# duckdb-faiss-ext/duckdb-faiss-ext

Hardware: AMD Instinct MI355X
Metric: queries/sec, FlatL2 d=128 N=10000000 nq=10000 k=10 (higher is better)
Workload: dtype f32 results (bf16 matrix-pipe coarse filter with a proven bound + exact f32 re-scoring of the candidates); 1 GPU; Flat L2 d=128 N=10000000 nq=10000 k=10; queries_per_call=10000, replicas=1, exchange=none

## Files before the change

### duckdb-faiss-ext_amd/csrc/common.h

```cpp
#pragma once
#include <hip/hip_runtime.h>

#include <cfloat>
#include <cstdint>
#include <cstdio>
#include <stdexcept>
#include <string>

namespace mvs {

struct Error : std::runtime_error {
	explicit Error(const std::string &m) : std::runtime_error(m) {
	}
};

[[noreturn]] void throw_faiss(const char *func, const char *file, const char *fmt, ...);

void ensure_dynamic_lds(const void *kernel, size_t bytes);

#define MVS_HIP(expr)                                                                                                  \
	do {                                                                                                               \
		hipError_t e_ = (expr);                                                                                        \
		if (e_ != hipSuccess)                                                                                          \
			::mvs::throw_faiss(__func__, __FILE__, "HIP error %d (%s) in %s", (int)e_, hipGetErrorString(e_), #expr);  \
// ... 91 lines not shown
                      int64_t nq, const unsigned short *d_rows_bf, const float *d_norms, int64_t n, int64_t kp, float *d_pd,
                      int32_t *d_pi, unsigned *d_gthr, hipStream_t st);
void launch_rescore_verify(int metric, const float *d_ca, const int64_t *d_ci, int64_t nq, int kp, int kk, const float *d_x,
                           const FlatGeom &g, const float *d_vecs, const float *d_norms, const float *d_qn,
                           const unsigned *d_max_norm_bits, float *d_pd1, int32_t *d_pi1, int *d_fail_cnt, int *d_fail_q,
                           unsigned *d_max_rel_err_bits, hipStream_t st);
void launch_gather_query_rows(const float *d_x, int d, const int *d_fq, int nf, float *d_xf, hipStream_t st);
void launch_scatter_rows(const int *d_fq, int nf, int64_t k, const float *d_Df, const int64_t *d_If, float *d_D,
                         int64_t *d_I, hipStream_t st);

constexpr int CL_OUTL_CAP = 256;
struct IvfFlatArith {
	const float *qn;
	const float *yn;
	const long long *rowids;
};

struct Tuning {
	int coarse_mfma = 2;
	int coarse_select = 1;
	int coarse_bf16 = 1;
	int cl_bound_mode = 1;
	int cl_tab = 1;
	int mfma_nsplit = 0;
	int mfma_global_lists = 1;
	int ivf_cl_xcd = 1;
};
const Tuning &tune();
void set_current_tuning(const Tuning *t);
void forget_current_tuning(const Tuning *t);

void trace_push(const char *name);
void trace_pop();
struct TraceRange {
	explicit TraceRange(const char *name) {
		trace_push(name);
	}
	~TraceRange() {
		trace_pop();
	}
	TraceRange(const TraceRange &) = delete;
	TraceRange &operator=(const TraceRange &) = delete;
};

struct DirectPlan {
	int nsplit;
// ... 106 lines not shown
```

### duckdb-faiss-ext_amd/csrc/flat_collect.h

```cpp
#pragma once
#include "flat_fused.h"

namespace mvs {

typedef __bf16 bf16x8 __attribute__((ext_vector_type(8)));
typedef float f32x4n __attribute__((ext_vector_type(4)));
typedef float f32x2n __attribute__((ext_vector_type(2)));
typedef int i32x4n __attribute__((ext_vector_type(4)));
typedef int i32x2n __attribute__((ext_vector_type(2)));
typedef __attribute__((address_space(3))) float lds_f32c;
typedef __attribute__((address_space(1))) const float glb_f32c;

constexpr int CL_QBLOCK = 512;
constexpr int CL_BN = 32;
constexpr double CL_MFMA_UNITS = 8.0;
constexpr int CL_SUB = 2;
constexpr int CL_QCAP = 2048;
constexpr int CL_FLUSH_EVERY = 2;
constexpr int CL_FROZEN = 256;

struct CollectArgs {
	const void *qf;
	const unsigned short *yb;
	const float *yn;
	const float *e2;
	unsigned *gslot;
	unsigned long long *stream;
	unsigned long long *stream_cnt;
	float *stream_s;
	float *seed_stage;
	const unsigned long long *rowmask;
	long long stream_cap;
	int slot_stride, nclass;
	long long n, row_first, split_rows;
	long long split_len;
	int nq, nqb, nsplit, xcd_map;
	float *pbnd;
	int flags;
	float i8_unit;
};

__device__ __forceinline__ int cl_i8_thr(float p, float inv_unit) {
	const float t = ceilf(p * inv_unit);
	if (!(t == t) || t > 1073741824.f)
		return 0x7fffffff;
	if (t < -1073741824.f)
		return -0x7fffffff;
	return (int)t;
}

int collect_store_dims(int d);
int collect_wide_qblock(int dp1);
int collect_wide_slots(int dp1);
int collect_wide_max_classes(int dp1);
size_t collect_wide_lds_bytes(int dp1);
int collect_wide_block_rows(int dp1);
void launch_collect_wide_range(int dp1, int metric, bool collect, CollectArgs a, int64_t row_first, int64_t row_end,
                               int64_t nsplit_want, int64_t nq, hipStream_t st, int *grid_out, int *nsplit_out);
int collect_big_qblock(int dp1);
size_t collect_big_lds_bytes(int dp1);
void launch_collect_big(int dp1, int metric, bool collect, const CollectArgs &a, int grid, hipStream_t st);
void launch_rows_to_bf16_wide(int metric, const float *d_vecs, int sdp, int interleaved, int d, int dp1, int64_t row0, int64_t nrows,
                              const float *d_mu, unsigned short *d_bf, float *d_beta, const float *d_norms,
                              unsigned *d_max_norm_bits, hipStream_t st, int *d_outl);
void launch_collect_exact_wide(int metric, bool per_pair, unsigned long long *d_sorted, int64_t ncand, const float *d_x, int d,
                               const float *d_vecs, int sdp, int interleaved, const float *d_norms, const float *d_qn, hipStream_t st,
                               const unsigned long long *d_cnt = nullptr);

__device__ __forceinline__ unsigned skey(float s) {
	return ~f2key(s);
}
__device__ __forceinline__ float skey2f(unsigned k) {
	return key2f(~k);
// ... 4 lines not shown
```

### duckdb-faiss-ext_amd/csrc/flat_collect.hip

```cpp
#include "flat_collect.h"

#include <algorithm>
#include <climits>
#include <cmath>
#include <cstring>
#include <type_traits>

#include <rocprim/device/device_radix_sort.hpp>
#include <rocprim/device/device_segmented_radix_sort.hpp>

namespace mvs {

__global__ __launch_bounds__(256) void collect_colsum_kernel(const float *__restrict__ src, long long nrows, int dp,
                                                            int interleaved, float *__restrict__ sum) {
	const int g8 = dp / 8, rl = threadIdx.x / g8, c8 = threadIdx.x % g8, nrl = 256 / g8;
	float acc[8] = {0.f, 0.f, 0.f, 0.f, 0.f, 0.f, 0.f, 0.f};
	const long long r0 = (long long)blockIdx.x * 1024;
	__shared__ float red[256 * 8];
	const bool idle = rl >= nrl;
	for (long long r = r0 + rl; !idle && r < r0 + 1024 && r < nrows; r += nrl) {
		const float4 s0 = *(const float4 *)(src + (size_t)r * dp + c8 * 8);
		const float4 s1 = *(const float4 *)(src + (size_t)r * dp + c8 * 8 + 4);
		float v[8];
		if (!interleaved) {
// ... 319 lines not shown
}

__global__ void collect_pack_queries_kernel(const float *__restrict__ x, long long nq, int d, int nkb,
                                            const float *__restrict__ mu, float alpha, bf16x8 *__restrict__ qf,
                                            long long total) {
	const long long i = (long long)blockIdx.x * blockDim.x + threadIdx.x;
	if (i >= total)
		return;
	const int lane = (int)(i & 63);
	const long long t = i >> 6;
	const int kb = (int)(t % nkb);
	const long long qblk16 = t / nkb;
	const long long q = qblk16 * 16 + (lane & 15);
	bf16x8 hi;
#pragma unroll
	for (int e = 0; e < 8; ++e) {
		const int kk = kb * 32 + 8 * (lane >> 4) + e;
		hi[e] = (__bf16)((q < nq && kk < d) ? alpha * (x[q * d + kk] - mu[kk]) : 0.f);
	}
	qf[i] = hi;
}
size_t collect_qfrag_bytes(const FlatGeom &g, int64_t nq) {
	(void)g;
	const int64_t nblk16 = (nq + CL_QBLOCK - 1) / CL_QBLOCK * (CL_QBLOCK / 16);
	return (size_t)nblk16 * 4 * 64 * 16;
}
size_t collect_qfrag_bytes_ex(int dp1, int qblock, int64_t nq) {
	const int64_t nblk16 = (nq + qblock - 1) / qblock * (qblock / 16);
	return (size_t)nblk16 * (dp1 / 32) * 64 * 16;
}
void launch_collect_pack_queries_ex(int d, int dp1, int qblock, int metric, const float *d_x, int64_t nq, const float *d_mu,
                                    void *d_qf, hipStream_t st) {
	const int64_t nblk16 = (nq + qblock - 1) / qblock * (qblock / 16);
	const long long total = (long long)nblk16 * (dp1 / 32) * 64;
	hipLaunchKernelGGL(collect_pack_queries_kernel, dim3((unsigned)((total + 255) / 256)), dim3(256), 0, st, d_x,
	                   (long long)nq, d, dp1 / 32, d_mu, metric == METRIC_L2 ? 2.0f : 1.0f, (bf16x8 *)d_qf, total);
	MVS_HIP(hipGetLastError());
}

template <bool IS_L2>
__global__ void collect_bounds_kernel(const float *__restrict__ x, long long nq, int d, const float *__restrict__ mu,
                                      const unsigned *__restrict__ max_norm_bits, float *__restrict__ e2,
                                      int *__restrict__ fail_cnt, int *__restrict__ fail_q, int bound_mode) {
	const long long q = (long long)blockIdx.x * blockDim.x + threadIdx.x;
	if (q >= nq) {
		e2[q] = __uint_as_float(0x7fc00000u);
		return;
// ... 173 lines not shown
			const int kk = kb * 32 + 8 * (lane >> 4) + e;
			hi[e] = (__bf16)((q0 + r < nq && kk < d) ? alpha * (xs[r][kk] - ms[kk]) : 0.f);
		}
		qf[((q0 / 16 + qb) * 4 + kb) * 64 + lane] = hi;
	}
	const unsigned neutral = ~f2key(-FLT_MAX);
	for (int i = tid; i < 64 * stride; i += 256) {
		const long long q = q0 + i / stride;
		if (q < nq)
			gslot[q * stride + (i % stride)] = neutral;
	}
	if (tid < 64 && q0 + tid < nq) {
		ctl_seg[q0 + tid] = 0;
		ctl_seg[nq + q0 + tid] = 0;
	}
	if (blockIdx.x == 0 && tid < 64)
		ctl_hdr[tid] = 0;
}
void launch_collect_query_prep(int metric, const float *d_x, int64_t nq, int d, const float *d_mu, const unsigned *d_max_norm_bits,
                               void *d_qf, float *d_qn, float *d_e2, int *d_fail_cnt, int *d_fail_q, unsigned *d_gslot, int stride,
                               int *d_ctl_hdr, int *d_ctl_seg, hipStream_t st, const unsigned *d_i8_bits, float i8_sa, float i8_unit) {
	if (nq <= 0)
		return;
	const long long nq_frag = (nq + CL_QBLOCK - 1) / CL_QBLOCK * CL_QBLOCK, nq_e2 = (nq + 255) / 256 * 256;
	const dim3 grid((unsigned)(nq_frag / 64));
	const bool i8 = i8_unit > 0.f;
	auto kern = metric == METRIC_L2 ? (i8 ? collect_query_prep_kernel<true, true> : collect_query_prep_kernel<true>)
	                                : (i8 ? collect_query_prep_kernel<false, true> : collect_query_prep_kernel<false>);
	hipLaunchKernelGGL(kern, grid, dim3(256), 0, st, d_x, (long long)nq, d, d_mu, d_max_norm_bits, (bf16x8 *)d_qf, nq_frag, d_qn, d_e2, nq_e2,
	                   d_fail_cnt, d_fail_q, tune().cl_bound_mode, d_gslot, stride, d_ctl_hdr, d_ctl_seg, d_i8_bits, i8_sa, i8_unit);
	MVS_HIP(hipGetLastError());
}

typedef float f32x4acc __attribute__((ext_vector_type(4)));
template <int KCH, bool IS_L2, bool COLLECT, bool SEL = false, int NC = 16, bool I8 = false>
__global__ __launch_bounds__(256, 2) void flat_bf16_collect_kernel(const CollectArgs a) {
	constexpr int DP = KCH * 16;
	constexpr int KB = I8 ? DP / 64 : DP / 32;
	constexpr int PITCH = I8 ? DP : DP * 2;
	constexpr int C = PITCH / 16;
	constexpr int TILE_BYTES = CL_BN * PITCH;
	constexpr int STAGE_BYTES = CL_SUB * TILE_BYTES;
	constexpr int NDMA = STAGE_BYTES / 1024;
	constexpr int DMA_PER_WAVE = NDMA / 4;
	static_assert(C == (I8 ? 8 : 16) && KB == (I8 ? 2 : 4) && NDMA % 4 == 0 && CL_SUB * CL_BN <= 64, "d = 128 geometry");
	typedef typename std::conditional<I8, i32x4n, bf16x8>::type frag_t;
	typedef typename std::conditional<I8, i32x4n, f32x4acc>::type acc_t;
	typedef typename std::conditional<I8, i32x2n, f32x2n>::type bnd_t;
	typedef typename std::conditional<I8, int, float>::type val_t;
	const float unit = a.i8_unit;

	extern __shared__ __attribute__((aligned(16))) float smem[];
	char *tbuf = (char *)smem;
	float *nbuf = (float *)(tbuf + 2 * STAGE_BYTES);
	unsigned long long *qbuf = (unsigned long long *)(nbuf + 2 * 64);
	float *cqtab = (float *)(qbuf + CL_QCAP);
	unsigned *qctl = (unsigned *)(cqtab + CL_QBLOCK);
	float *qval = (float *)(qctl + 16);
	float *cqstage = qval + CL_QCAP;

	const int tid = threadIdx.x, lane = tid & 63;
	const int wave = __builtin_amdgcn_readfirstlane(tid >> 6);
	const int hq = lane >> 4, c = lane & 15;
	int split, qb;
	if (a.xcd_map) {
		const int xcd = blockIdx.x & 7, idx = blockIdx.x >> 3;
		split = (idx / a.nqb) * 8 + xcd;
		qb = idx % a.nqb;
	} else {
		split = blockIdx.x / a.nqb;
		qb = blockIdx.x % a.nqb;
	}
	const long long r_begin = a.row_first + (long long)split * a.split_rows;
	long long r_end = r_begin + a.split_rows;
	if (r_end > a.n)
		r_end = a.n;
	const int ntiles = r_end > r_begin ? (int)((r_end - r_begin + CL_SUB * CL_BN - 1) / (CL_SUB * CL_BN)) : 0;
	if (tid == 0)
		qctl[7] = 0u;

	const int qw = qb * CL_QBLOCK + wave * 128;

	frag_t bq[8][KB];
	{
		const frag_t *qsrc = (const frag_t *)a.qf;
#pragma unroll
		for (int cb = 0; cb < 8; ++cb) {
			const size_t qblk16 = (size_t)qb * (CL_QBLOCK / 16) + wave * 8 + cb;
#pragma unroll
			for (int kb = 0; kb < KB; ++kb)
				bq[cb][kb] = qsrc[(qblk16 * KB + kb) * 64 + lane];
		}
	}

	unsigned dma_off;
	{
		const int rr = I8 ? 8 * wave + (lane >> 3) : 4 * wave + (lane >> 4);
		dma_off = (unsigned)(rr * PITCH + (((lane & (C - 1)) ^ (rr & (C - 1))) * 16));
	}
	auto dma_issue = [&](int u, int i) {
		const char *base = (const char *)a.yb + (size_t)(r_begin + (long long)u * (CL_SUB * CL_BN)) * PITCH + (size_t)i * 4096;
		__builtin_amdgcn_global_load_lds((glb_f32c *)(base + dma_off),
		                                 (lds_f32c *)(smem + ((u & 1) * STAGE_BYTES + (i * 4 + wave) * 1024) / 4), 16, 0, 0);
	};
	auto dma_norms = [&](int u) {
		const float *base = a.yn + (r_begin + (long long)u * (CL_SUB * CL_BN));
		__builtin_amdgcn_global_load_lds((glb_f32c *)(base + lane), (lds_f32c *)(smem + (2 * STAGE_BYTES) / 4 + (u & 1) * 64),
		                                 4, 0, 0);
	};
	const bool use_tab = a.pbnd != nullptr;
	const bool frozen = use_tab && (a.flags & CL_FROZEN) != 0;
	constexpr int tab_shift = 2;
	constexpr int duty_mask = !COLLECT ? 3 : (NC > 32 ? 255 : 63);
	const int duty_phase = split * 13 + 5;
	bool tab_pending = false;
	const float inv_unit = I8 ? 1.0f / unit : 0.f;
	auto dma_bounds = [&]() {
		const float *base = a.pbnd + (size_t)qb * CL_QBLOCK + wave * 128;
		float *dst = (I8 ? cqstage : cqtab) + wave * 128;
		__builtin_amdgcn_global_load_lds((glb_f32c *)(base + lane), (lds_f32c *)dst, 4, 0, 16 );
		__builtin_amdgcn_global_load_lds((glb_f32c *)(base + 64 + lane), (lds_f32c *)(dst + 64), 4, 0, 16);
		tab_pending = I8;
	};
	auto tab_cvt = [&]() {
		if (!I8 || !tab_pending)
			return;
		tab_pending = false;
		const float p0 = cqstage[wave * 128 + lane], p1 = cqstage[wave * 128 + 64 + lane];
		((int *)cqtab)[wave * 128 + lane] = cl_i8_thr(p0, inv_unit);
		((int *)cqtab)[wave * 128 + 64 + lane] = cl_i8_thr(p1, inv_unit);
	};
	if (ntiles > 0) {
#pragma unroll
		for (int i = 0; i < DMA_PER_WAVE; ++i)
			dma_issue(0, i);
		dma_norms(0);
		if (use_tab)
			dma_bounds();
	}
	__syncthreads();
	tab_cvt();

	const unsigned rbase = (unsigned)(c * PITCH) | (unsigned)(((hq ^ c) & (C - 1)) * 16);
	constexpr int WQCAP = CL_QCAP / 4;
	const unsigned qcnt_lds = (unsigned)(uintptr_t)((__attribute__((address_space(3))) unsigned *)qctl);
	const unsigned qbuf_lds = (unsigned)(uintptr_t)((__attribute__((address_space(3))) unsigned long long *)qbuf) + (unsigned)(wave * WQCAP * 8);
	const unsigned qval_lds = (unsigned)(uintptr_t)((__attribute__((address_space(3))) float *)qval) + (unsigned)(wave * WQCAP * 4);
	const unsigned cq_lds = (unsigned)(uintptr_t)((__attribute__((address_space(3))) float *)cqtab) + (unsigned)((wave * 64 + c) * 8);

	int ovf = 0;
	int wfill = 0, wpub = 0;
	auto publish = [&]() __attribute__((always_inline)) {
		const unsigned n = (unsigned)wfill < (unsigned)WQCAP ? (unsigned)wfill : (unsigned)WQCAP;
		for (unsigned e = (unsigned)wpub + lane; e < n && !frozen; e += 64) {
			unsigned long long ent;
			float v;
			asm volatile("ds_read_b64 %0, %2\n\tds_read_b32 %1, %3\n\ts_waitcnt lgkmcnt(0)"
			             : "=&v"(ent), "=&v"(v)
			             : "v"(qbuf_lds + 8u * e), "v"(qval_lds + 4u * e)
			             : "memory");
			const unsigned row = (unsigned)ent;
			typedef __attribute__((address_space(1))) unsigned *GU;
			__hip_atomic_fetch_min((GU)(a.gslot + (size_t)(unsigned)(ent >> 32) * NC) + (row & (unsigned)(NC - 1)), skey(v), __ATOMIC_RELAXED,
			                       __HIP_MEMORY_SCOPE_AGENT);
		}
		wpub = (int)n;
	};
	auto wdrain = [&]() __attribute__((always_inline)) {
		publish();
		const unsigned n = (unsigned)wpub;
		wfill = 0;
// ... 69 lines not shown
				const unsigned long long ent = ((unsigned long long)q << 32) | row;
				if (__builtin_expect(!counting, 1)) {
					asm volatile("ds_write_b64 %0, %1\n\tds_write_b32 %2, %3" ::"v"(qbuf_lds + 8u * pos), "v"(ent), "v"(qval_lds + 4u * pos), "v"(v) : "memory");
				} else {
					typedef __attribute__((address_space(1))) unsigned *GU;
					__hip_atomic_fetch_min((GU)(a.gslot + (size_t)q * NC) + (row & (unsigned)(NC - 1)), skey(v), __ATOMIC_RELAXED,
					                       __HIP_MEMORY_SCOPE_AGENT);
					const unsigned one = 1u;
					asm volatile("ds_add_u32 %0, %1" ::"v"(qcnt_lds + 28u), "v"(one) : "memory");
				}
			}
		}
	};

	for (int u = 0; u < ntiles; ++u) {
		const int period = u < 4 ? 1 : (u < 32 ? 8 : (u < 256 ? 32 : 128));
		const bool full = !frozen && (use_tab ? ((u + duty_phase) & duty_mask) == 0 : (u % period) == 0);
		if (use_tab && !full && u > 0 && (u & ((1 << tab_shift) - 1)) == 0)
			dma_bounds();
		if (full) {
			publish();
			int qo = qw;
			MVS_OPAQUE_VGPR(qo);
			f32x2n v = {0.f, 0.f};
#pragma unroll 1
			for (int i = 0; i < 2; ++i) {
				const int q = qo + 32 * hq + 16 * i + c;
				const int qc = q < a.nq ? q : 0;
				const float e2v = __builtin_nontemporal_load(a.e2 + qc);
				constexpr int SUBN = NC > 32 ? 32 : NC, NSUB = NC / SUBN;
				const int rank = NSUB == 1 ? a.nclass - 1 : (a.nclass + NSUB - 1) / NSUB - 1;
				unsigned kth = 0u;
#pragma unroll 1
				for (int sb = 0; sb < NSUB; ++sb) {
				const unsigned long long *src = (const unsigned long long *)(a.gslot + (size_t)qc * NC + sb * SUBN);
				unsigned long long w[SUBN / 2];
#pragma unroll
				for (int j = 0; j < SUBN / 2; ++j)
					w[j] = __hip_atomic_load(src + j, __ATOMIC_RELAXED, __HIP_MEMORY_SCOPE_AGENT);
#pragma unroll
				for (int j = 0; j < SUBN / 2; ++j)
					asm volatile("" : "+v"(w[j]));
				unsigned key[SUBN];
#pragma unroll
				for (int j = 0; j < SUBN / 2; ++j) {
					key[2 * j] = (unsigned)w[j];
					key[2 * j + 1] = (unsigned)(w[j] >> 32);
				}
#pragma unroll
				for (int kbit = 2; kbit <= SUBN; kbit <<= 1)
// ... 4 lines not shown
							const int x1 = x0 ^ jb;
							if (x1 > x0) {
								const unsigned lo = key[x0] < key[x1] ? key[x0] : key[x1];
								const unsigned hi = key[x0] < key[x1] ? key[x1] : key[x0];
								const bool asc = (x0 & kbit) == 0;
								key[x0] = asc ? lo : hi;
								key[x1] = asc ? hi : lo;
							}
						}
				unsigned ks = key[0];
#pragma unroll
				for (int j = 1; j < SUBN; ++j)
					ks = (rank == j) ? key[j] : ks;
				kth = ks > kth ? ks : kth;
				}
				const unsigned neutral = skey(-FLT_MAX);
				const float B = skey2f(kth < neutral ? kth : neutral);
				const float bv = q < a.nq ? B - e2v : __uint_as_float(0x7fc00000u);
				v[0] = i == 0 ? bv : v[0];
				v[1] = i == 1 ? bv : v[1];
			}
			if (I8) {
				const i32x2n vi = {cl_i8_thr(v[0], inv_unit), cl_i8_thr(v[1], inv_unit)};
				*(i32x2n *)(cqtab + (wave * 64 + hq * 16 + c) * 2) = vi;
			} else {
				*(f32x2n *)(cqtab + (wave * 64 + hq * 16 + c) * 2) = v;
			}
			if (use_tab) {
				unsigned long long bits;
				__builtin_memcpy(&bits, &v, 8);
				__hip_atomic_store((unsigned long long *)(a.pbnd + (size_t)qb * CL_QBLOCK + (wave * 64 + hq * 16 + c) * 2), bits, __ATOMIC_RELAXED,
				                   __HIP_MEMORY_SCOPE_AGENT);
			}
		}
#pragma unroll 1
		for (int sub = 0; sub < CL_SUB; ++sub) {
		frag_t A[KB][2];
		acc_t Y[2];
		{
			const unsigned nb_lds = (unsigned)(uintptr_t)((lds_f32c *)(nbuf + (u & 1) * 64 + sub * CL_BN + 4 * hq));
			asm volatile("ds_read_b128 %0, %2\n\tds_read_b128 %1, %2 offset:64" : "=&v"(Y[0]), "=&v"(Y[1]) : "v"(nb_lds) : "memory");
			const unsigned ab =
			    (unsigned)(uintptr_t)((lds_f32c *)(smem + ((u & 1) * STAGE_BYTES + sub * TILE_BYTES) / 4)) + rbase;
#pragma unroll
			for (int kb = 0; kb < KB; ++kb) {
				asm volatile("ds_read_b128 %0, %1" : "=v"(A[kb][0]) : "v"(ab ^ (unsigned)(kb * 64)) : "memory");
				if (I8)
					asm volatile("ds_read_b128 %0, %1 offset:2048" : "=v"(A[kb][1]) : "v"(ab ^ (unsigned)(kb * 64)) : "memory");
				else
					asm volatile("ds_read_b128 %0, %1 offset:4096" : "=v"(A[kb][1]) : "v"(ab ^ (unsigned)(kb * 64)) : "memory");
			}
		}
		if (sub == 0) {
#pragma unroll
			for (int i = 0; i < DMA_PER_WAVE; ++i)
// ... 12 lines not shown
		bnd_t cqv[2];
		const val_t lowest = I8 ? (val_t)INT_MIN : (val_t)-INFINITY;
		val_t mx0 = lowest, mx1 = lowest;
		auto vmax = [](val_t x, val_t y) {
			if constexpr (I8)
				return x > y ? x : y;
			else
				return __builtin_fmaxf(x, y);
		};
		auto fold = [&](acc_t &p, int rb, int i) {
			(void)rb;
			if (i == 0)
				mx0 = vmax(vmax(vmax(vmax(mx0, p[0]), p[1]), p[2]), p[3]);
			else
				mx1 = vmax(vmax(vmax(vmax(mx1, p[0]), p[1]), p[2]), p[3]);
		};
		auto any_of = [&](bnd_t cqp) {
			const bool r = (mx0 >= cqp[0]) || (mx1 >= cqp[1]);
			mx0 = lowest;
			mx1 = lowest;
			return r;
		};
#pragma unroll
		for (int t = 0; t < 4; ++t) {
			asm volatile("ds_read_b64 %0, %1" : "=v"(cqv[t & 1]) : "v"(cq_lds + (unsigned)(t * 128)) : "memory");
#pragma unroll
			for (int rb = 0; rb < 2; ++rb) {
				const int prb = rb ^ 1, pt = rb == 0 ? t - 1 : t;
#pragma unroll
				for (int kb = 0; kb < KB; ++kb) {
					if constexpr (I8) {
						if (t == 0) {
							if (rb == 0 && kb == 0)
								asm volatile("s_waitcnt lgkmcnt(4)" : "+v"(A[0][0]), "+v"(Y[0]), "+v"(Y[1]));
							else if (rb == 0 && kb == 1)
								asm volatile("s_waitcnt lgkmcnt(2)" : "+v"(A[1][0]));
							else if (rb == 1 && kb == 0)
								asm volatile("s_waitcnt lgkmcnt(0)" : "+v"(A[0][1]), "+v"(A[1][1]), "+v"(cqv[0]));
						}
					} else if (t == 0) {
						if (rb == 0 && kb == 0)
							asm volatile("s_waitcnt lgkmcnt(8)" : "+v"(A[0][0]), "+v"(Y[0]), "+v"(Y[1]));
						else if (rb == 0 && kb == 1)
							asm volatile("s_waitcnt lgkmcnt(6)" : "+v"(A[1][0]));
						else if (rb == 0 && kb == 2)
							asm volatile("s_waitcnt lgkmcnt(4)" : "+v"(A[2][0]));
						else if (rb == 0 && kb == 3)
// ... 4 lines not shown
#pragma unroll
					for (int i = 0; i < 2; ++i) {
						if constexpr (I8)
							acc[rb][i] = __builtin_amdgcn_mfma_i32_16x16x64_i8(A[kb][rb], bq[2 * t + i][kb], kb == 0 ? Y[rb] : acc[rb][i], 0, 0, 0);
						else if (kb == 0)
							acc[rb][i] = __builtin_amdgcn_mfma_f32_16x16x32_bf16(A[kb][rb], bq[2 * t + i][kb], Y[rb], 0, 0, 0);
						else
							acc[rb][i] = __builtin_amdgcn_mfma_f32_16x16x32_bf16(A[kb][rb], bq[2 * t + i][kb], acc[rb][i], 0, 0, 0);
					}
					if (pt >= 0 && kb < 2)
						fold(acc[prb][kb], prb, kb);
					__builtin_amdgcn_sched_barrier(0);
				}
				if (pt >= 0) {
					if (rb == 0)
						asm volatile("s_waitcnt lgkmcnt(0)" : "+v"(cqv[0]), "+v"(cqv[1]));
					rare(acc[prb], prb, pt, any_of(cqv[pt & 1]), cqv[pt & 1], row0, nvalid, rowbits);
				}
			}
		}
		{
			fold(acc[1][0], 1, 0);
			fold(acc[1][1], 1, 1);
			rare(acc[1], 1, 3, any_of(cqv[1]), cqv[1], row0, nvalid, rowbits);
		}
		}
		__syncthreads();
		tab_cvt();
		if ((u % CL_FLUSH_EVERY) == CL_FLUSH_EVERY - 1 || u == ntiles - 1) {
			if (wfill >= WQCAP / 2 || u == ntiles - 1)
				wdrain();
			else
				publish();
		}
	}
	if (COLLECT) {
		__syncthreads();
		if (tid == 0 && qctl[7] != 0u)
			atomicAdd(a.stream_cnt, (unsigned long long)qctl[7]);
	}
}

static size_t collect_lds_bytes(const FlatGeom &g, bool i8) {
	(void)g;
	return (size_t)2 * CL_SUB * CL_BN * 128 * (i8 ? 1 : 2) + 2 * 64 * 4 + (size_t)CL_QCAP * 8 + (size_t)CL_QBLOCK * 4 + 64 + (size_t)CL_QCAP * 4 +
	       (i8 ? (size_t)CL_QBLOCK * 4 : 0);
}

bool collect_supported(const FlatGeom &g) {
	return collect_store_dims(g.d) > 0;
}

__device__ __forceinline__ bool cl_sel_member(const SelectorDev &s, long long id) {
	if (s.kind == MVS_SEL_BITMAP) {
		const unsigned long long u = (unsigned long long)id;
		if ((u >> 3) >= (unsigned long long)s.nbytes)
			return false;
		return (s.bitmap[u >> 3] >> (u & 7)) & 1;
	}
	if (s.kind == MVS_SEL_BATCH) {
		long long lo = 0, hi = s.nids;
		while (lo < hi) {
			const long long mid = (lo + hi) >> 1;
			if (s.sorted_ids[mid] < id)
				lo = mid + 1;
			else
				hi = mid;
		}
		return lo < s.nids && s.sorted_ids[lo] == id;
// ... 7 lines not shown
	if (row < n)
		ok = cl_sel_member(sel, idmap ? idmap[row] : row);
	const unsigned long long b = __builtin_amdgcn_ballot_w64(ok);
	if ((threadIdx.x & 63) == 0 && (row >> 6) < nwords)
		mask[row >> 6] = b;
}
size_t collect_rowmask_bytes(int64_t n) {
	return (size_t)((n + 63) / 64 + 64) * 8;
}
void launch_collect_rowmask(SelectorDev sel, const int64_t *d_idmap, int64_t n, unsigned long long *d_mask, hipStream_t st) {
	const long long nwords = (long long)(collect_rowmask_bytes(n) / 8);
	const long long rows = nwords * 64;
	hipLaunchKernelGGL(collect_rowmask_kernel, dim3((unsigned)((rows + 255) / 256)), dim3(256), 0, st, sel,
	                   (const long long *)d_idmap, (long long)n, nwords, d_mask);
	MVS_HIP(hipGetLastError());
}


int flat_mfma_slot_stride(int64_t k);
__global__ void init_gslot_kernel(unsigned *g, long long total, int stride, int k, int is_l2);

template <int NC>
__global__ void collect_bound_table_kernel(const unsigned *__restrict__ gslot, const float *__restrict__ e2, int nclass, int nq,
                                           long long total, float *__restrict__ pbnd) {
	const long long j = (long long)blockIdx.x * blockDim.x + threadIdx.x;
	if (j >= total)
		return;
	const int o = (int)(j & 127), w = (int)((j >> 7) & 3);
	const long long qb = j >> 9;
	const int i = o & 1, c = (o >> 1) & 15, hq = o >> 5;
	const long long q = qb * CL_QBLOCK + w * 128 + 32 * hq + 16 * i + c;
	float bv = __uint_as_float(0x7fc00000u);
	if (q < nq) {
		constexpr int SUBN = NC > 32 ? 32 : NC, NSUB = NC / SUBN;
		const int rank = NSUB == 1 ? nclass - 1 : (nclass + NSUB - 1) / NSUB - 1;
		unsigned kth = 0u;
		for (int sb = 0; sb < NSUB; ++sb) {
			unsigned key[SUBN];
#pragma unroll
			for (int t = 0; t < SUBN; ++t)
				key[t] = gslot[(size_t)q * NC + sb * SUBN + t];
			unsigned ks = 0xffffffffu;
#pragma unroll
			for (int t = 0; t < SUBN; ++t) {
				int less = 0, leq = 0;
#pragma unroll
				for (int s2 = 0; s2 < SUBN; ++s2) {
					less += key[s2] < key[t];
					leq += key[s2] <= key[t];
				}
				if (less <= rank && rank < leq)
					ks = key[t];
			}
			kth = ks > kth ? ks : kth;
		}
		const unsigned neutral = skey(-FLT_MAX);
		const float B = skey2f(kth < neutral ? kth : neutral);
		bv = B - e2[q];
	}
	pbnd[j] = bv;
}
static void launch_collect_bound_table(const CollectArgs &a, int nqb, hipStream_t st) {
	if (!a.pbnd)
		return;
	const long long total = (long long)nqb * CL_QBLOCK;
	const dim3 grid((unsigned)((total + 255) / 256));
	if (a.slot_stride == 128)
		hipLaunchKernelGGL(collect_bound_table_kernel<128>, grid, dim3(256), 0, st, (const unsigned *)a.gslot, a.e2, a.nclass, a.nq, total, a.pbnd);
	else if (a.slot_stride == 32)
		hipLaunchKernelGGL(collect_bound_table_kernel<32>, grid, dim3(256), 0, st, (const unsigned *)a.gslot, a.e2, a.nclass, a.nq, total, a.pbnd);
	else
		hipLaunchKernelGGL(collect_bound_table_kernel<16>, grid, dim3(256), 0, st, (const unsigned *)a.gslot, a.e2, a.nclass, a.nq, total, a.pbnd);
	MVS_HIP(hipGetLastError());
}
size_t collect_bound_table_bytes(int64_t nq) {
	return (size_t)((nq + CL_QBLOCK - 1) / CL_QBLOCK) * CL_QBLOCK * sizeof(float) + 1024;
}

template <bool COLLECT>
static void launch_collect_range(const FlatGeom &g, int metric, CollectArgs a, int64_t row_first, int64_t row_end,
                                 int64_t nsplit_want, int64_t nq, hipStream_t st, int *grid_out, int *nsplit_out) {
	const int nqb = (int)((nq + CL_QBLOCK - 1) / CL_QBLOCK);
	if (!tune().cl_tab && !(a.flags & CL_FROZEN))
		a.pbnd = nullptr;
	if (!(a.flags & CL_FROZEN))
		launch_collect_bound_table(a, nqb, st);
	const int64_t ntiles = (row_end - row_first + CL_SUB * CL_BN - 1) / (CL_SUB * CL_BN);
	const int64_t nsplit = std::max<int64_t>(1, std::min<int64_t>(nsplit_want, ntiles));
	a.xcd_map = (nsplit >= 8 && nsplit % 8 == 0) ? 1 : 0;
	a.row_first = row_first;
	a.n = row_end;
	a.split_rows = (ntiles + nsplit - 1) / nsplit * (CL_SUB * CL_BN);
	a.nqb = nqb;
	a.nsplit = (int)nsplit;
	const int grid = nqb * (int)nsplit;
	const bool i8 = a.i8_unit > 0.f;
	const size_t lds = collect_lds_bytes(g, i8);
#define MVS_CL_GO(L2, SEL_, NC_)                                                                                        \
	{                                                                                                                  \
		auto kern = i8 ? flat_bf16_collect_kernel<8, L2, COLLECT, SEL_, NC_, true> : flat_bf16_collect_kernel<8, L2, COLLECT, SEL_, NC_>; \
		ensure_dynamic_lds((const void *)kern, lds);                                                                   \
		hipLaunchKernelGGL(kern, dim3(grid), dim3(256), lds, st, a);                                                   \
	}
	if (a.slot_stride == 32 || a.slot_stride == 128) {
#define MVS_CL_NC32(L2, SEL_)                                                                                           \
	{                                                                                                                  \
		if (a.slot_stride == 128)                                                                                      \
			MVS_CL_GO(L2, SEL_, 128)                                                                                   \
		else                                                                                                           \
			MVS_CL_GO(L2, SEL_, 32)                                                                                    \
	}
		if (a.rowmask && metric == METRIC_L2)
			MVS_CL_NC32(true, true)
		else if (a.rowmask)
			MVS_CL_NC32(false, true)
		else if (metric == METRIC_L2)
			MVS_CL_NC32(true, false)
		else
			MVS_CL_NC32(false, false)
#undef MVS_CL_NC32
	} else if (a.rowmask) {
		if (metric == METRIC_L2)
			MVS_CL_GO(true, true, 16)
		else
			MVS_CL_GO(false, true, 16)
	} else if (metric == METRIC_L2) {
		MVS_CL_GO(true, false, 16)
	} else {
		MVS_CL_GO(false, false, 16)
	}
#undef MVS_CL_GO
	MVS_HIP(hipGetLastError());
	if (grid_out)
		*grid_out = grid;
	if (nsplit_out)
		*nsplit_out = (int)nsplit;
}


template <bool IS_L2, bool SEL, bool I8 = false>
__global__ __launch_bounds__(256, 2) void flat_bf16_seed_kernel(const CollectArgs a) {
	constexpr int KB = I8 ? 2 : 4, PITCH = I8 ? 128 : 256, C = PITCH / 16;
	constexpr int TILE_BYTES = CL_BN * PITCH, STAGE_BYTES = CL_SUB * TILE_BYTES;
	constexpr int DMA_PER_WAVE = STAGE_BYTES / 4096;
	typedef typename std::conditional<I8, i32x4n, bf16x8>::type frag_t;
	typedef typename std::conditional<I8, i32x4n, f32x4acc>::type acc_t;
	typedef typename std::conditional<I8, int, float>::type val_t;
	const val_t lowest = I8 ? (val_t)INT_MIN : (val_t)-INFINITY;
// ... 216 lines not shown
#pragma unroll
		for (int t = 0; t < SUBN; ++t) {
			int less = 0, leq = 0;
#pragma unroll
			for (int s2 = 0; s2 < SUBN; ++s2) {
				less += key[s2] < key[t];
				leq += key[s2] <= key[t];
			}
			if (less <= rank && rank < leq)
				ks = key[t];
		}
		kth = ks > kth ? ks : kth;
	}
	const unsigned neutral = skey(-FLT_MAX);
	const float B = skey2f(kth < neutral ? kth : neutral);
	thr[q] = B - e2[q];
}
__global__ void collect_bound_table_multi_kernel(const unsigned *__restrict__ gslot, long long range_stride, int nranges,
                                                 const float *__restrict__ e2, int nclass, int nq, long long total, float *__restrict__ pbnd,
                                                 int linear) {
	const long long j = (long long)blockIdx.x * blockDim.x + threadIdx.x;
	if (j >= total)
		return;
	const int o = (int)(j & 127), w = (int)((j >> 7) & 3);
	const long long qb = j >> 9;
	const int i = o & 1, c = (o >> 1) & 15, hq = o >> 5;
	const long long q = linear ? j : qb * CL_QBLOCK + w * 128 + 32 * hq + 16 * i + c;
	float bv = __uint_as_float(0x7fc00000u);
	if (q < nq) {
		const int rank = (nclass + 3) / 4 - 1;
		unsigned kth = 0u;
		for (int p = 0; p < nranges; ++p)
			for (int sb = 0; sb < 4; ++sb) {
				unsigned key[32];
#pragma unroll
				for (int t = 0; t < 32; ++t)
					key[t] = gslot[(size_t)p * range_stride + (size_t)q * 128 + sb * 32 + t];
				unsigned ks = 0xffffffffu;
#pragma unroll
				for (int t = 0; t < 32; ++t) {
					int less = 0, leq = 0;
#pragma unroll
					for (int s2 = 0; s2 < 32; ++s2) {
						less += key[s2] < key[t];
						leq += key[s2] <= key[t];
					}
					if (less <= rank && rank < leq)
						ks = key[t];
				}
				kth = ks > kth ? ks : kth;
			}
		const unsigned neutral = skey(-FLT_MAX);
		const float B = skey2f(kth < neutral ? kth : neutral);
		bv = B - e2[q];
	}
	pbnd[j] = bv;
}
__global__ void collect_bound_table_seed_kernel(const float *__restrict__ stage, int nsplit, int rank, const float *__restrict__ e2, int nq,
                                                long long total, float *__restrict__ pbnd) {
	const long long j = (long long)blockIdx.x * blockDim.x + threadIdx.x;
	if (j >= total)
		return;
	const int o = (int)(j & 127), w = (int)((j >> 7) & 3);
	const long long qb = j >> 9;
	const int i = o & 1, c = (o >> 1) & 15, hq = o >> 5;
	const long long q = qb * CL_QBLOCK + w * 128 + 32 * hq + 16 * i + c;
	float bv = __uint_as_float(0x7fc00000u);
	if (q < nq) {
		float T = INFINITY;
		for (int p = 0; p < nsplit; ++p) {
			float v[16];
			const f32x4acc *src = (const f32x4acc *)(stage + ((size_t)p * (size_t)nq + (size_t)q) * 16);
#pragma unroll
			for (int t = 0; t < 4; ++t) {
				const f32x4acc x = src[t];
				v[4 * t] = x[0], v[4 * t + 1] = x[1], v[4 * t + 2] = x[2], v[4 * t + 3] = x[3];
			}
			float b = -INFINITY;
#pragma unroll
			for (int t = 0; t < 16; ++t) {
				const float vt = v[t] == v[t] ? v[t] : -INFINITY;
				int greater = 0, geq = 0;
#pragma unroll
				for (int s2 = 0; s2 < 16; ++s2) {
					const float vs = v[s2] == v[s2] ? v[s2] : -INFINITY;
					greater += vs > vt;
					geq += vs >= vt;
				}
				if (greater <= rank && rank < geq)
// ... 141 lines not shown
	a.pbnd = d_pbnd;
	const int dp1 = collect_store_dims(g.d);
	a.i8_unit = dp1 > 128 ? 0.f : i8_unit;
	if (dp1 == 128 && stride == 16) {
		constexpr int64_t seed_reg_rows = 32768;
		const int64_t rows = std::min<int64_t>(seed_reg_rows, n / 8) / 64 * 64;
		if (rows >= 1024) {
			a.seed_stage = d_seed_stage;
			launch_collect_seed(metric, a, rows, nq, st);
		}
		return;
	}
	constexpr int64_t seed_rows = 16384, seed_split = 32;
	const int64_t kscale = std::max(1, kk / 16);
	const int64_t seed = std::min<int64_t>(n, kscale * std::min<int64_t>(seed_rows, std::max<int64_t>(2048, n / 256)));
	if (seed > 0 && seed < n) {
		if (dp1 > 128)
			launch_collect_wide_range(dp1, metric, false, a, 0, seed, seed_split, nq, st, nullptr, nullptr);
		else
			launch_collect_range<false>(g, metric, a, 0, seed, seed_split, nq, st, nullptr, nullptr);
	}
}

void launch_collect_scan(const FlatGeom &g, int metric, const void *d_qf, const unsigned short *d_rows, const float *d_norms,
                         int64_t n, int64_t nq, int kk, const float *d_e2, unsigned *d_gslot, unsigned long long *d_stream,
                         unsigned long long *d_stream_cnt, int64_t stream_cap, const unsigned long long *d_rowmask, float *d_pbnd,
                         hipStream_t st, int *grid_out, int *nsplit_out, int *lds_out, float *d_stream_s, bool frozen, float i8_unit) {
	CollectArgs a;
	memset(&a, 0, sizeof a);
	a.qf = d_qf;
	a.yb = d_rows;
	a.yn = d_norms;
	a.e2 = d_e2;
	a.gslot = d_gslot;
	a.slot_stride = frozen ? 16 : collect_slot_stride(kk, collect_store_dims(g.d));
	a.nclass = frozen ? 16 : kk;
	a.nq = (int)nq;
	a.stream = d_stream;
	a.stream_s = d_stream_s;
	a.stream_cnt = d_stream_cnt;
	a.stream_cap = stream_cap;
	a.rowmask = d_rowmask;
	a.flags = frozen ? CL_FROZEN : 0;
	a.pbnd = d_pbnd;
	const int dp1 = collect_store_dims(g.d);
	a.i8_unit = dp1 > 128 ? 0.f : i8_unit;
	const int qblock = dp1 > 128 ? collect_wide_qblock(dp1) : CL_QBLOCK;
	const int nqb = (int)((nq + qblock - 1) / qblock);
	const int64_t slots = dp1 > 128 ? collect_wide_slots(dp1) : 512;
	const int64_t max_split = std::max<int64_t>(1, n / 7680);
	int64_t nsplit = 1;
	double best = -1;
	for (int64_t s = 8; s <= std::min<int64_t>(max_split, 512); s += 8) {
		const int64_t w = s * nqb, rounds = (w + slots - 1) / slots;
		double eff = (double)w / (double)(rounds * slots);
		if (rounds < 2)
			eff -= 0.05;
		eff += 1e-5 * (double)std::min<int64_t>(rounds, 10);
		if (eff > best) {
			best = eff;
			nsplit = s;
		}
	}
	if (max_split < 8)
		nsplit = max_split;
	if (dp1 > 128)
		launch_collect_wide_range(dp1, metric, true, a, 0, n, nsplit, nq, st, grid_out, nsplit_out);
	else
		launch_collect_range<true>(g, metric, a, 0, n, nsplit, nq, st, grid_out, nsplit_out);
	if (lds_out)
		*lds_out = (int)(dp1 > 128 ? collect_wide_lds_bytes(dp1) : collect_lds_bytes(g, a.i8_unit > 0.f));
}

__global__ void collect_count_queries_kernel(const unsigned long long *__restrict__ stream, long long n, int *__restrict__ qcount) {
	const long long i = (long long)blockIdx.x * blockDim.x + threadIdx.x;
	if (i < n)
		atomicAdd(&qcount[(unsigned)(stream[i] >> 32)], 1);
}
__global__ void collect_drop_heavy_kernel(const int *__restrict__ qcount, long long nq, int share, float *__restrict__ e2,
                                          int *__restrict__ fail_cnt, int *__restrict__ fail_q, int *__restrict__ nheavy) {
	const long long q = (long long)blockIdx.x * blockDim.x + threadIdx.x;
	if (q >= nq || qcount[q] <= share || e2[q] != e2[q])
		return;
	e2[q] = __uint_as_float(0x7fc00000u);
	fail_q[atomicAdd(fail_cnt, 1)] = (int)q;
	atomicAdd(nheavy, 1);
}
int launch_collect_drop_heavy(const unsigned long long *d_stream, int64_t n, int64_t nq, int share, int *d_qcount ,
                              float *d_e2, int *d_fail_cnt, int *d_fail_q, hipStream_t st) {
	hipLaunchKernelGGL(collect_count_queries_kernel, dim3((unsigned)((n + 255) / 256)), dim3(256), 0, st, d_stream, (long long)n, d_qcount);
	hipLaunchKernelGGL(collect_drop_heavy_kernel, dim3((unsigned)((nq + 255) / 256)), dim3(256), 0, st, (const int *)d_qcount,
	                   (long long)nq, share, d_e2, d_fail_cnt, d_fail_q, d_qcount + nq);
	MVS_HIP(hipGetLastError());
	int nheavy = 0;
// ... 485 lines not shown
```

### duckdb-faiss-ext_amd/csrc/index.hip

```cpp
#include "index.h"

#include <atomic>
#include <condition_variable>
#include <map>
#include <mutex>
#include <thread>

#include <algorithm>
#include <dlfcn.h>
#include <chrono>
#include <cstdarg>
#include <cstdlib>
#include <cstring>

namespace mvs {

static thread_local std::string g_last_error;

void throw_faiss(const char *func, const char *file, const char *fmt, ...) {
	char msg[512];
	va_list ap;
	va_start(ap, fmt);
	vsnprintf(msg, sizeof msg, fmt, ap);
	va_end(ap);
// ... 2677 lines not shown
	static const Tuning defaults;
	return t_tune ? *t_tune : defaults;
}
void set_current_tuning(const Tuning *t) {
	t_tune = t;
}
void forget_current_tuning(const Tuning *t) {
	if (t_tune == t)
		t_tune = nullptr;
}
bool IndexBase::set_tuning(const char *key, int64_t v) {
	struct Key {
		const char *name;
		int Tuning::*field;
		bool flag;
	};
	static const Key keys[] = {
	    {"ivf_coarse_mfma", &Tuning::coarse_mfma, false},
	    {"ivf_cl_xcd", &Tuning::ivf_cl_xcd, false},
	    {"ivf_coarse_select", &Tuning::coarse_select, true},
	    {"ivf_coarse_bf16", &Tuning::coarse_bf16, true},
	    {"cl_bound_mode", &Tuning::cl_bound_mode, false},
	    {"cl_tab", &Tuning::cl_tab, true},
	    {"mfma_global_lists", &Tuning::mfma_global_lists, false},
	    {"mfma_nsplit", &Tuning::mfma_nsplit, false},
	};
	for (const Key &e : keys) {
		if (strcmp(key, e.name))
			continue;
		tune_.*(e.field) = e.flag ? v != 0 : (int)v;
		return true;
	}
	return false;
}
bool FlatIndex::set_option(const char *key, int64_t v) {
	if (set_tuning(key, v))
		return true;
	if (!strcmp(key, "cl_i8")) {
		cl_i8 = v != 0;
		return true;
	}
	if (!strcmp(key, "outlier_rows")) {
		outlier_rows = v != 0;
		return true;
	}
	if (!strcmp(key, "lazy_adds")) {
// ... 77 lines not shown
```

Before: 872,600 queries/s.

## Let each wave hold 256 queries in the int8 coarse collect scan

Adds a QW template parameter to the bf16/int8 collect kernel so one wave can keep 256 query fragments in registers instead of 128, making a block cover 1024 queries. Each streamed database tile is then reused against twice as many queries, which halves row re-reads and tile staging per query. Bound tables, LDS layout, query-fragment indexing and buffer sizing are generalised through new helper functions. A selector (cl_qw) picks 256 only for the int8, 16-slot, non-frozen, non-masked path when the padding overhead is small. The trade-off is much higher register pressure under launch_bounds(256,2), with a risk of spills or lower occupancy, plus fewer blocks per split.

```diff
diff --git a/duckdb-faiss-ext_amd/csrc/common.h b/duckdb-faiss-ext_amd/csrc/common.h
--- a/duckdb-faiss-ext_amd/csrc/common.h
+++ b/duckdb-faiss-ext_amd/csrc/common.h
@@ -137,6 +137,7 @@
 	int coarse_bf16 = 1;
 	int cl_bound_mode = 1;
 	int cl_tab = 1;
+	int cl_qw = 1;
 	int mfma_nsplit = 0;
 	int mfma_global_lists = 1;
 	int ivf_cl_xcd = 1;
diff --git a/duckdb-faiss-ext_amd/csrc/flat_collect.h b/duckdb-faiss-ext_amd/csrc/flat_collect.h
--- a/duckdb-faiss-ext_amd/csrc/flat_collect.h
+++ b/duckdb-faiss-ext_amd/csrc/flat_collect.h
@@ -12,6 +12,7 @@
 typedef __attribute__((address_space(1))) const float glb_f32c;
 
 constexpr int CL_QBLOCK = 512;
+constexpr int CL_QBLOCK_MAX = 1024;
 constexpr int CL_BN = 32;
 constexpr double CL_MFMA_UNITS = 8.0;
 constexpr int CL_SUB = 2;
@@ -49,6 +50,18 @@
 	return (int)t;
 }
 
+__host__ __device__ inline long long cl_query_of(long long qb, int qw, int w, int t, int i, int c) {
+	return qb * 4 * qw + (long long)w * qw + 32 * t + 16 * i + c;
+}
+__host__ __device__ inline long long cl_tab_query(long long j, int qw) {
+	const int o = (int)(j % qw), w = (int)((j / qw) & 3);
+	return cl_query_of(j / (4 * qw), qw, w, o >> 5, o & 1, (o >> 1) & 15);
+}
+__host__ __device__ inline long long cl_frag_block(long long qb, int qw, int w, int cb) {
+	return qb * (4 * qw / 16) + (long long)w * (qw / 16) + cb;
+}
+int collect_scan_qw(int64_t nq, int slot_stride, bool selector, bool frozen, bool i8);
+
 int collect_store_dims(int d);
 int collect_wide_qblock(int dp1);
 int collect_wide_slots(int dp1);
diff --git a/duckdb-faiss-ext_amd/csrc/flat_collect.hip b/duckdb-faiss-ext_amd/csrc/flat_collect.hip
--- a/duckdb-faiss-ext_amd/csrc/flat_collect.hip
+++ b/duckdb-faiss-ext_amd/csrc/flat_collect.hip
@@ -365,7 +365,7 @@
 }
 size_t collect_qfrag_bytes(const FlatGeom &g, int64_t nq) {
 	(void)g;
-	const int64_t nblk16 = (nq + CL_QBLOCK - 1) / CL_QBLOCK * (CL_QBLOCK / 16);
+	const int64_t nblk16 = (nq + CL_QBLOCK_MAX - 1) / CL_QBLOCK_MAX * (CL_QBLOCK_MAX / 16);
 	return (size_t)nblk16 * 4 * 64 * 16;
 }
 size_t collect_qfrag_bytes_ex(int dp1, int qblock, int64_t nq) {
@@ -585,7 +585,7 @@
                                int *d_ctl_hdr, int *d_ctl_seg, hipStream_t st, const unsigned *d_i8_bits, float i8_sa, float i8_unit) {
 	if (nq <= 0)
 		return;
-	const long long nq_frag = (nq + CL_QBLOCK - 1) / CL_QBLOCK * CL_QBLOCK, nq_e2 = (nq + 255) / 256 * 256;
+	const long long nq_frag = (nq + CL_QBLOCK_MAX - 1) / CL_QBLOCK_MAX * CL_QBLOCK_MAX, nq_e2 = (nq + 255) / 256 * 256;
 	const dim3 grid((unsigned)(nq_frag / 64));
 	const bool i8 = i8_unit > 0.f;
 	auto kern = metric == METRIC_L2 ? (i8 ? collect_query_prep_kernel<true, true> : collect_query_prep_kernel<true>)
@@ -596,9 +596,13 @@
 }
 
 typedef float f32x4acc __attribute__((ext_vector_type(4)));
-template <int KCH, bool IS_L2, bool COLLECT, bool SEL = false, int NC = 16, bool I8 = false>
+template <int KCH, bool IS_L2, bool COLLECT, bool SEL = false, int NC = 16, bool I8 = false, int QW = 128>
 __global__ __launch_bounds__(256, 2) void flat_bf16_collect_kernel(const CollectArgs a) {
 	constexpr int DP = KCH * 16;
+	constexpr int QB = 4 * QW;
+	constexpr int NT = QW / 32;
+	constexpr int NCB = QW / 16;
+	static_assert(QW == 128 || (QW == 256 && I8), "256 queries per wave: the int8 fragments only (16 x 2 x 4 = 128 registers)");
 	constexpr int KB = I8 ? DP / 64 : DP / 32;
 	constexpr int PITCH = I8 ? DP : DP * 2;
 	constexpr int C = PITCH / 16;
@@ -618,7 +622,7 @@
 	float *nbuf = (float *)(tbuf + 2 * STAGE_BYTES);
 	unsigned long long *qbuf = (unsigned long long *)(nbuf + 2 * 64);
 	float *cqtab = (float *)(qbuf + CL_QCAP);
-	unsigned *qctl = (unsigned *)(cqtab + CL_QBLOCK);
+	unsigned *qctl = (unsigned *)(cqtab + QB);
 	float *qval = (float *)(qctl + 16);
 	float *cqstage = qval + CL_QCAP;
 
@@ -642,14 +646,14 @@
 	if (tid == 0)
 		qctl[7] = 0u;
 
-	const int qw = qb * CL_QBLOCK + wave * 128;
-
-	frag_t bq[8][KB];
+	const int qw = qb * QB + wave * QW;
+
+	frag_t bq[NCB][KB];
 	{
 		const frag_t *qsrc = (const frag_t *)a.qf;
 #pragma unroll
-		for (int cb = 0; cb < 8; ++cb) {
-			const size_t qblk16 = (size_t)qb * (CL_QBLOCK / 16) + wave * 8 + cb;
+		for (int cb = 0; cb < NCB; ++cb) {
+			const size_t qblk16 = (size_t)cl_frag_block(qb, QW, wave, cb);
 #pragma unroll
 			for (int kb = 0; kb < KB; ++kb)
 				bq[cb][kb] = qsrc[(qblk16 * KB + kb) * 64 + lane];
@@ -679,19 +683,20 @@
 	bool tab_pending = false;
 	const float inv_unit = I8 ? 1.0f / unit : 0.f;
 	auto dma_bounds = [&]() {
-		const float *base = a.pbnd + (size_t)qb * CL_QBLOCK + wave * 128;
-		float *dst = (I8 ? cqstage : cqtab) + wave * 128;
-		__builtin_amdgcn_global_load_lds((glb_f32c *)(base + lane), (lds_f32c *)dst, 4, 0, 16 );
-		__builtin_amdgcn_global_load_lds((glb_f32c *)(base + 64 + lane), (lds_f32c *)(dst + 64), 4, 0, 16);
+		const float *base = a.pbnd + (size_t)qb * QB + wave * QW;
+		float *dst = (I8 ? cqstage : cqtab) + wave * QW;
+#pragma unroll
+		for (int p = 0; p < QW / 64; ++p)
+			__builtin_amdgcn_global_load_lds((glb_f32c *)(base + 64 * p + lane), (lds_f32c *)(dst + 64 * p), 4, 0, 16);
 		tab_pending = I8;
 	};
 	auto tab_cvt = [&]() {
 		if (!I8 || !tab_pending)
 			return;
 		tab_pending = false;
-		const float p0 = cqstage[wave * 128 + lane], p1 = cqstage[wave * 128 + 64 + lane];
-		((int *)cqtab)[wave * 128 + lane] = cl_i8_thr(p0, inv_unit);
-		((int *)cqtab)[wave * 128 + 64 + lane] = cl_i8_thr(p1, inv_unit);
+#pragma unroll
+		for (int p = 0; p < QW / 64; ++p)
+			((int *)cqtab)[wave * QW + 64 * p + lane] = cl_i8_thr(cqstage[wave * QW + 64 * p + lane], inv_unit);
 	};
 	if (ntiles > 0) {
 #pragma unroll
@@ -709,7 +714,7 @@
 	const unsigned qcnt_lds = (unsigned)(uintptr_t)((__attribute__((address_space(3))) unsigned *)qctl);
 	const unsigned qbuf_lds = (unsigned)(uintptr_t)((__attribute__((address_space(3))) unsigned long long *)qbuf) + (unsigned)(wave * WQCAP * 8);
 	const unsigned qval_lds = (unsigned)(uintptr_t)((__attribute__((address_space(3))) float *)qval) + (unsigned)(wave * WQCAP * 4);
-	const unsigned cq_lds = (unsigned)(uintptr_t)((__attribute__((address_space(3))) float *)cqtab) + (unsigned)((wave * 64 + c) * 8);
+	const unsigned cq_lds = (unsigned)(uintptr_t)((__attribute__((address_space(3))) float *)cqtab) + (unsigned)((wave * (QW / 2) + c) * 8);
 
 	int ovf = 0;
 	int wfill = 0, wpub = 0;
@@ -825,10 +830,12 @@
 			publish();
 			int qo = qw;
 			MVS_OPAQUE_VGPR(qo);
+#pragma unroll 1
+			for (int to = hq; to < NT; to += 4) {
 			f32x2n v = {0.f, 0.f};
 #pragma unroll 1
 			for (int i = 0; i < 2; ++i) {
-				const int q = qo + 32 * hq + 16 * i + c;
+				const int q = qo + 32 * to + 16 * i + c;
 				const int qc = q < a.nq ? q : 0;
 				const float e2v = __builtin_nontemporal_load(a.e2 + qc);
 				constexpr int SUBN = NC > 32 ? 32 : NC, NSUB = NC / SUBN;
@@ -879,15 +886,16 @@
 			}
 			if (I8) {
 				const i32x2n vi = {cl_i8_thr(v[0], inv_unit), cl_i8_thr(v[1], inv_unit)};
-				*(i32x2n *)(cqtab + (wave * 64 + hq * 16 + c) * 2) = vi;
+				*(i32x2n *)(cqtab + (wave * (QW / 2) + to * 16 + c) * 2) = vi;
 			} else {
-				*(f32x2n *)(cqtab + (wave * 64 + hq * 16 + c) * 2) = v;
+				*(f32x2n *)(cqtab + (wave * (QW / 2) + to * 16 + c) * 2) = v;
 			}
 			if (use_tab) {
 				unsigned long long bits;
 				__builtin_memcpy(&bits, &v, 8);
-				__hip_atomic_store((unsigned long long *)(a.pbnd + (size_t)qb * CL_QBLOCK + (wave * 64 + hq * 16 + c) * 2), bits, __ATOMIC_RELAXED,
+				__hip_atomic_store((unsigned long long *)(a.pbnd + (size_t)qb * QB + (wave * (QW / 2) + to * 16 + c) * 2), bits, __ATOMIC_RELAXED,
 				                   __HIP_MEMORY_SCOPE_AGENT);
+			}
 			}
 		}
 #pragma unroll 1
@@ -946,7 +954,7 @@
 			return r;
 		};
 #pragma unroll
-		for (int t = 0; t < 4; ++t) {
+		for (int t = 0; t < NT; ++t) {
 			asm volatile("ds_read_b64 %0, %1" : "=v"(cqv[t & 1]) : "v"(cq_lds + (unsigned)(t * 128)) : "memory");
 #pragma unroll
 			for (int rb = 0; rb < 2; ++rb) {
@@ -997,7 +1005,7 @@
 		{
 			fold(acc[1][0], 1, 0);
 			fold(acc[1][1], 1, 1);
-			rare(acc[1], 1, 3, any_of(cqv[1]), cqv[1], row0, nvalid, rowbits);
+			rare(acc[1], 1, NT - 1, any_of(cqv[(NT - 1) & 1]), cqv[(NT - 1) & 1], row0, nvalid, rowbits);
 		}
 		}
 		__syncthreads();
@@ -1016,10 +1024,10 @@
 	}
 }
 
-static size_t collect_lds_bytes(const FlatGeom &g, bool i8) {
+static size_t collect_lds_bytes(const FlatGeom &g, bool i8, int qw = 128) {
 	(void)g;
-	return (size_t)2 * CL_SUB * CL_BN * 128 * (i8 ? 1 : 2) + 2 * 64 * 4 + (size_t)CL_QCAP * 8 + (size_t)CL_QBLOCK * 4 + 64 + (size_t)CL_QCAP * 4 +
-	       (i8 ? (size_t)CL_QBLOCK * 4 : 0);
+	return (size_t)2 * CL_SUB * CL_BN * 128 * (i8 ? 1 : 2) + 2 * 64 * 4 + (size_t)CL_QCAP * 8 + (size_t)4 * qw * 4 + 64 + (size_t)CL_QCAP * 4 +
+	       (i8 ? (size_t)4 * qw * 4 : 0);
 }
 
 bool collect_supported(const FlatGeom &g) {
@@ -1073,14 +1081,11 @@
 
 template <int NC>
 __global__ void collect_bound_table_kernel(const unsigned *__restrict__ gslot, const float *__restrict__ e2, int nclass, int nq,
-                                           long long total, float *__restrict__ pbnd) {
+                                           long long total, float *__restrict__ pbnd, int qw) {
 	const long long j = (long long)blockIdx.x * blockDim.x + threadIdx.x;
 	if (j >= total)
 		return;
-	const int o = (int)(j & 127), w = (int)((j >> 7) & 3);
-	const long long qb = j >> 9;
-	const int i = o & 1, c = (o >> 1) & 15, hq = o >> 5;
-	const long long q = qb * CL_QBLOCK + w * 128 + 32 * hq + 16 * i + c;
+	const long long q = cl_tab_query(j, qw);
 	float bv = __uint_as_float(0x7fc00000u);
 	if (q < nq) {
 		constexpr int SUBN = NC > 32 ? 32 : NC, NSUB = NC / SUBN;
@@ -1111,31 +1116,31 @@
 	}
 	pbnd[j] = bv;
 }
-static void launch_collect_bound_table(const CollectArgs &a, int nqb, hipStream_t st) {
+static void launch_collect_bound_table(const CollectArgs &a, int nqb, int qw, hipStream_t st) {
 	if (!a.pbnd)
 		return;
-	const long long total = (long long)nqb * CL_QBLOCK;
+	const long long total = (long long)nqb * 4 * qw;
 	const dim3 grid((unsigned)((total + 255) / 256));
 	if (a.slot_stride == 128)
-		hipLaunchKernelGGL(collect_bound_table_kernel<128>, grid, dim3(256), 0, st, (const unsigned *)a.gslot, a.e2, a.nclass, a.nq, total, a.pbnd);
+		hipLaunchKernelGGL(collect_bound_table_kernel<128>, grid, dim3(256), 0, st, (const unsigned *)a.gslot, a.e2, a.nclass, a.nq, total, a.pbnd, qw);
 	else if (a.slot_stride == 32)
-		hipLaunchKernelGGL(collect_bound_table_kernel<32>, grid, dim3(256), 0, st, (const unsigned *)a.gslot, a.e2, a.nclass, a.nq, total, a.pbnd);
+		hipLaunchKernelGGL(collect_bound_table_kernel<32>, grid, dim3(256), 0, st, (const unsigned *)a.gslot, a.e2, a.nclass, a.nq, total, a.pbnd, qw);
 	else
-		hipLaunchKernelGGL(collect_bound_table_kernel<16>, grid, dim3(256), 0, st, (const unsigned *)a.gslot, a.e2, a.nclass, a.nq, total, a.pbnd);
+		hipLaunchKernelGGL(collect_bound_table_kernel<16>, grid, dim3(256), 0, st, (const unsigned *)a.gslot, a.e2, a.nclass, a.nq, total, a.pbnd, qw);
 	MVS_HIP(hipGetLastError());
 }
 size_t collect_bound_table_bytes(int64_t nq) {
-	return (size_t)((nq + CL_QBLOCK - 1) / CL_QBLOCK) * CL_QBLOCK * sizeof(float) + 1024;
+	return (size_t)((nq + CL_QBLOCK_MAX - 1) / CL_QBLOCK_MAX) * CL_QBLOCK_MAX * sizeof(float) + 1024;
 }
 
 template <bool COLLECT>
 static void launch_collect_range(const FlatGeom &g, int metric, CollectArgs a, int64_t row_first, int64_t row_end,
-                                 int64_t nsplit_want, int64_t nq, hipStream_t st, int *grid_out, int *nsplit_out) {
-	const int nqb = (int)((nq + CL_QBLOCK - 1) / CL_QBLOCK);
+                                 int64_t nsplit_want, int64_t nq, hipStream_t st, int *grid_out, int *nsplit_out, int qw = 128) {
+	const int nqb = (int)((nq + 4 * qw - 1) / (4 * qw));
 	if (!tune().cl_tab && !(a.flags & CL_FROZEN))
 		a.pbnd = nullptr;
 	if (!(a.flags & CL_FROZEN))
-		launch_collect_bound_table(a, nqb, st);
+		launch_collect_bound_table(a, nqb, qw, st);
 	const int64_t ntiles = (row_end - row_first + CL_SUB * CL_BN - 1) / (CL_SUB * CL_BN);
 	const int64_t nsplit = std::max<int64_t>(1, std::min<int64_t>(nsplit_want, ntiles));
 	a.xcd_map = (nsplit >= 8 && nsplit % 8 == 0) ? 1 : 0;
@@ -1146,7 +1151,7 @@
 	a.nsplit = (int)nsplit;
 	const int grid = nqb * (int)nsplit;
 	const bool i8 = a.i8_unit > 0.f;
-	const size_t lds = collect_lds_bytes(g, i8);
+	const size_t lds = collect_lds_bytes(g, i8, qw);
 #define MVS_CL_GO(L2, SEL_, NC_)                                                                                        \
 	{                                                                                                                  \
 		auto kern = i8 ? flat_bf16_collect_kernel<8, L2, COLLECT, SEL_, NC_, true> : flat_bf16_collect_kernel<8, L2, COLLECT, SEL_, NC_>; \
@@ -1175,6 +1180,13 @@
 			MVS_CL_GO(true, true, 16)
 		else
 			MVS_CL_GO(false, true, 16)
+	} else if (qw == 256) {
+		if constexpr (COLLECT) {
+			auto kern = metric == METRIC_L2 ? flat_bf16_collect_kernel<8, true, true, false, 16, true, 256>
+			                                : flat_bf16_collect_kernel<8, false, true, false, 16, true, 256>;
+			ensure_dynamic_lds((const void *)kern, lds);
+			hipLaunchKernelGGL(kern, dim3(grid), dim3(256), lds, st, a);
+		}
 	} else if (metric == METRIC_L2) {
 		MVS_CL_GO(true, false, 16)
 	} else {
@@ -1437,10 +1449,7 @@
 	const long long j = (long long)blockIdx.x * blockDim.x + threadIdx.x;
 	if (j >= total)
 		return;
-	const int o = (int)(j & 127), w = (int)((j >> 7) & 3);
-	const long long qb = j >> 9;
-	const int i = o & 1, c = (o >> 1) & 15, hq = o >> 5;
-	const long long q = linear ? j : qb * CL_QBLOCK + w * 128 + 32 * hq + 16 * i + c;
+	const long long q = linear ? j : cl_tab_query(j, 128);
 	float bv = __uint_as_float(0x7fc00000u);
 	if (q < nq) {
 		const int rank = (nclass + 3) / 4 - 1;
@@ -1476,10 +1485,7 @@
 	const long long j = (long long)blockIdx.x * blockDim.x + threadIdx.x;
 	if (j >= total)
 		return;
-	const int o = (int)(j & 127), w = (int)((j >> 7) & 3);
-	const long long qb = j >> 9;
-	const int i = o & 1, c = (o >> 1) & 15, hq = o >> 5;
-	const long long q = qb * CL_QBLOCK + w * 128 + 32 * hq + 16 * i + c;
+	const long long q = cl_tab_query(j, 128);
 	float bv = __uint_as_float(0x7fc00000u);
 	if (q < nq) {
 		float T = INFINITY;
@@ -1667,6 +1673,16 @@
 	}
 }
 
+int collect_scan_qw(int64_t nq, int slot_stride, bool selector, bool frozen, bool i8) {
+	const int mode = tune().cl_qw;
+	if (!i8 || slot_stride != 16 || selector || frozen || mode == 0)
+		return 128;
+	if (mode >= 2)
+		return 256;
+	const int64_t pad512 = (nq + 511) / 512 * 512, pad1024 = (nq + 1023) / 1024 * 1024;
+	return pad1024 * 16 <= pad512 * 17 ? 256 : 128;
+}
+
 void launch_collect_scan(const FlatGeom &g, int metric, const void *d_qf, const unsigned short *d_rows, const float *d_norms,
                          int64_t n, int64_t nq, int kk, const float *d_e2, unsigned *d_gslot, unsigned long long *d_stream,
                          unsigned long long *d_stream_cnt, int64_t stream_cap, const unsigned long long *d_rowmask, float *d_pbnd,
@@ -1690,7 +1706,8 @@
 	a.pbnd = d_pbnd;
 	const int dp1 = collect_store_dims(g.d);
 	a.i8_unit = dp1 > 128 ? 0.f : i8_unit;
-	const int qblock = dp1 > 128 ? collect_wide_qblock(dp1) : CL_QBLOCK;
+	const int qw = dp1 > 128 ? 128 : collect_scan_qw(nq, a.slot_stride, d_rowmask != nullptr, frozen, a.i8_unit > 0.f);
+	const int qblock = dp1 > 128 ? collect_wide_qblock(dp1) : 4 * qw;
 	const int nqb = (int)((nq + qblock - 1) / qblock);
 	const int64_t slots = dp1 > 128 ? collect_wide_slots(dp1) : 512;
 	const int64_t max_split = std::max<int64_t>(1, n / 7680);
@@ -1712,9 +1729,9 @@
 	if (dp1 > 128)
 		launch_collect_wide_range(dp1, metric, true, a, 0, n, nsplit, nq, st, grid_out, nsplit_out);
 	else
-		launch_collect_range<true>(g, metric, a, 0, n, nsplit, nq, st, grid_out, nsplit_out);
+		launch_collect_range<true>(g, metric, a, 0, n, nsplit, nq, st, grid_out, nsplit_out, qw);
 	if (lds_out)
-		*lds_out = (int)(dp1 > 128 ? collect_wide_lds_bytes(dp1) : collect_lds_bytes(g, a.i8_unit > 0.f));
+		*lds_out = (int)(dp1 > 128 ? collect_wide_lds_bytes(dp1) : collect_lds_bytes(g, a.i8_unit > 0.f, qw));
 }
 
 __global__ void collect_count_queries_kernel(const unsigned long long *__restrict__ stream, long long n, int *__restrict__ qcount) {
diff --git a/duckdb-faiss-ext_amd/csrc/index.hip b/duckdb-faiss-ext_amd/csrc/index.hip
--- a/duckdb-faiss-ext_amd/csrc/index.hip
+++ b/duckdb-faiss-ext_amd/csrc/index.hip
@@ -2723,6 +2723,7 @@
 	    {"ivf_coarse_bf16", &Tuning::coarse_bf16, true},
 	    {"cl_bound_mode", &Tuning::cl_bound_mode, false},
 	    {"cl_tab", &Tuning::cl_tab, true},
+	    {"cl_qw", &Tuning::cl_qw, false},
 	    {"mfma_global_lists", &Tuning::mfma_global_lists, false},
 	    {"mfma_nsplit", &Tuning::mfma_nsplit, false},
 	};
```

Measured after the change: 963,300 queries/s, median of 6. 10.4% higher.
